# jamesonquinn/Mamba.jl

Hardware: AMD Instinct MI355X
Metric: chain-updates/sec (iters×chains) on rats model at 1/2/4/8 MI355X (higher is better)
Workload: dtype f64

## Files before the change

### mamba.jl_amd/csrc/device.h

```cpp
#pragma once
#if !defined(__HIPCC_RTC__)
#include <hip/hip_runtime.h>
#include <stdint.h>
#endif

#include "mamba_hip.h"
#include "mmb_math.h"
#include "ir_math.h"

#define MMB_MAXB MMB_MAX_BLOCKS

__device__ __forceinline__ bool mmb_inverse_ballot(uint64_t m) {
#if defined(__HIPCC_RTC__)
  return ((m >> (threadIdx.x & 63)) & 1ull) != 0ull;
#else
  return __builtin_amdgcn_inverse_ballot_w64(m);
#endif
}

template <bool B>
struct mmb_bc {
  static constexpr bool value = B;
  constexpr operator bool() const { return B; }
};
// ... 38 lines not shown
  double* t_accept;
  int32_t* t_m;
  int32_t* t_flags;
  double* t_Mv;
  double* t_Mvv;
  double* t_Ls;
  uint8_t* t_piv;
  double* t_xnext;
  int64_t* t_xtag;
  uint64_t* t_astat;
  double* t_nuts;
  double* t_nfr;
  double* t_hmc;
  int32_t ir_blk;
  int32_t fdgrad;
  const int32_t* sep;
  double sep_eps;
  int32_t gibbs_fam;
  double gibbs_a;
};

struct SweepArgs {
  int32_t K;
  uint32_t chain_offset;
  uint64_t seed;
  int64_t iter0;
  int32_t n_iters;
  int32_t nb;
  int64_t burnin, thin, model_burnin;
  int64_t kept_base;
  int64_t kept_origin;
  double* vals;
  int64_t xepoch;
  unsigned long long* nuts_stat;
  double* draws;
  const double* data0;
  double ig_c;
  double xbar;
  double xm[5];
  double lx[5], ly[5];
  const DBlock* blocks;
  const mmb_ir_node* ir_nodes;
  const int32_t* ir_code;
  const double* ir_const;
  const double* ir_pool;
  const mmb_ir_block* ir_blocks;
  const int32_t* ir_mon;
  int32_t ir_nmon, ir_pmon;
  int32_t ir_vs;
  int32_t ir_red0;
  int32_t ir_amm;
  int32_t ir_lds;
  const int32_t* cperm;
  int32_t amwg_exact;
  int32_t slice_exact;
  int32_t amwg_probe;
};

#define MMB_ORDER_BLOCKS 3
struct OrderArgs {
  const int32_t* flags[MMB_ORDER_BLOCKS];
  int32_t nblk;
  int32_t K;
  int32_t cpw;
  int32_t mode;
  int32_t* perm;
};

__device__ __forceinline__ const DBlock& mmb_block(const DBlock* p, int b) {
#if defined(__HIP_DEVICE_COMPILE__)
  return *(const DBlock*)&((const __attribute__((address_space(4))) DBlock*)p)[b];
#else
  return p[b];
#endif
}

MMB_HD int mmb_tri(int i) { return (i * (i + 1)) >> 1; }
MMB_HD int mmb_slot(int i, int k) { return i >= k ? mmb_tri(i) + k : mmb_tri(k) + i; }

__device__ __forceinline__ void grp_sync() {
  __builtin_amdgcn_fence(__ATOMIC_RELEASE, "wavefront");
  __builtin_amdgcn_wave_barrier();
  __builtin_amdgcn_fence(__ATOMIC_ACQUIRE, "wavefront");
}

template <int CTRL>
__device__ __forceinline__ int dpp_i(int x) {
  return __builtin_amdgcn_mov_dpp(x, CTRL, 0xF, 0xF, true);
}
template <int CTRL>
__device__ __forceinline__ double dpp_d(double x) {
  uint64_t u = mmb_d2u(x);
  int lo = dpp_i<CTRL>((int)(uint32_t)u), hi = dpp_i<CTRL>((int)(uint32_t)(u >> 32));
  return mmb_u2d((uint64_t)(uint32_t)lo | ((uint64_t)(uint32_t)hi << 32));
}
__device__ __forceinline__ int swap16_i(int x) {
  auto r = __builtin_amdgcn_permlane16_swap((unsigned)x, (unsigned)x, false, false);
  return (int)((threadIdx.x & 16) ? r[0] : r[1]);
}
__device__ __forceinline__ double swap16_d(double x) {
  uint64_t u = mmb_d2u(x);
  int lo = swap16_i((int)(uint32_t)u), hi = swap16_i((int)(uint32_t)(u >> 32));
  return mmb_u2d((uint64_t)(uint32_t)lo | ((uint64_t)(uint32_t)hi << 32));
}
template <int N, bool FIRST>
__device__ __forceinline__ void fmac_rowbc(double& acc, double x, double b) {
// ... 176 lines not shown
```

### mamba.jl_amd/csrc/engine.cpp

```cpp
#include <hip/hip_runtime.h>

#include <algorithm>
#include <cmath>
#include <cstdarg>
#include <cstdio>
#include <cstdlib>
#include <cstring>
#include <map>
#include <string>
#include <type_traits>
#include <vector>

#include "device.h"
#include "models.h"
#include "nuts.h"
#include "logistic.h"
#include "ir.h"
#include "ir_jit.h"

#include <rccl/rccl.h>

hipError_t mmb_launch_sweep(int model, unsigned kinds, const SweepArgs& A, hipStream_t st);
hipError_t mmb_launch_order_chains(const OrderArgs& a, hipStream_t st);
hipError_t mmb_launch_pchol_probe(int n, int d, const double* S, double* L, int32_t* pos, int32_t* info,
                                  hipStream_t st);
hipError_t mmb_lg_launch_ctl(const LgArgs& A, int start, int parity, int nbound, int fold, hipStream_t st);
hipError_t mmb_lg_launch_grad(const LgArgs& A, int parity, int nbound, int fold, hipStream_t st);
hipError_t mmb_launch_gr_range(int pmon, int64_t n, int K, const double* draws, double* out,
                               hipStream_t st);
hipError_t mmb_launch_chain_summary(int P, int64_t n, int K, int64_t kg0, int64_t bs, const double* draws,
                                    const double* shift, double* out, hipStream_t st);
hipError_t mmb_launch_order_hist(int P, int j, int64_t n, int K, const double* draws, int nt,
                                 const uint64_t* prefix, int pass, unsigned long long* counts, hipStream_t st);
hipError_t mmb_launch_gr_stats(int pmon, int64_t n, int K, const double* draws, const int32_t* link,
                               const double* shift, double* stats, hipStream_t st);

static thread_local std::string g_last_error;

struct BlockHost {
  mmb_block_spec spec;
  std::vector<double> tuning;
  int d = 0, T = 0, tune_len = 0;
  std::vector<double> sigl;
  bool sigl_diag = false;
  double *sigma = nullptr, *accept = nullptr, *Mv = nullptr, *Mvv = nullptr, *Ls = nullptr;
  double *nuts = nullptr, *nfr = nullptr, *width = nullptr, *sigl_d = nullptr;
  double* hmc = nullptr;
  int32_t *m = nullptr, *flags = nullptr;
  uint8_t* piv = nullptr;
  double* xnext = nullptr;
  int64_t* xtag = nullptr;
  uint64_t* astat = nullptr;
  int32_t* sep_d = nullptr;
  double sep_eps = 0.0;
};

struct mmb_engine {
  mmb_model_spec spec{};
  int device = 0;
  hipStream_t stream = nullptr;
  int model = 0;
  int P = 0, pmon = 0, VS = 0, DP = 0, TP = 0;
  std::vector<BlockHost> blocks;
  unsigned kinds = 0;
  std::vector<double> x, y, X;
  bool have_data = false;
  double* d_data = nullptr;
  int64_t K = 0, chain_offset = 0;
  uint64_t seed = 0;
  int64_t iter = 0;
  double* d_vals = nullptr;
  DBlock* d_blocks = nullptr;
  int lg_N = 0, lg_p = 0, lg_rps = 0;
  bool lg_fd = false;
  double *lg_X = nullptr, *lg_y = nullptr;
  double *lg_vec = nullptr, *lg_sc = nullptr, *lg_frames = nullptr, *lg_pos = nullptr;
  double *lg_gpart = nullptr, *lg_lpart = nullptr;
  int32_t *lg_iv = nullptr, *lg_count = nullptr, *lg_hcount = nullptr, *lg_s2c = nullptr;
  int64_t* lg_itc = nullptr;
  hipEvent_t lg_cev[2 * MMB_LG_SPLIT_MAX] = {};
  hipStream_t lg_streamx[MMB_LG_SPLIT_MAX - 1] = {};
  hipEvent_t lg_join[MMB_LG_SPLIT_MAX] = {};
  std::vector<hipEvent_t> evpoolx[MMB_LG_SPLIT_MAX - 1];
  int64_t lg_steps = 0;
  unsigned long long* lg_ngrad = nullptr;
  int32_t* d_cperm = nullptr;
  bool cperm_identity = true;
  bool order_fresh = false;
  int64_t order_iter = 0;
  unsigned long long* d_nstat = nullptr;
  unsigned long long slice_overflows = 0;
  int64_t xepoch = 0;
  double* d_draws = nullptr;
  size_t draws_cap = 0;
  int64_t n_kept = 0;
  std::vector<mmb_ir_node> ir_nodes;
  std::vector<int32_t> ir_code, ir_mon;
  std::vector<double> ir_const, ir_pool;
  std::vector<mmb_ir_block> ir_blocks;
  int ir_stack = 0;
  mmb_ir_node* d_ir_nodes = nullptr;
  int32_t *d_ir_code = nullptr, *d_ir_mon = nullptr;
  double *d_ir_const = nullptr, *d_ir_pool = nullptr;
  mmb_ir_block* d_ir_blocks = nullptr;
  hipModule_t jit_mod = nullptr;
  hipFunction_t jit_fn = nullptr;
  bool ir_noprop = false;
  int ir_stack_dbl = 0;
  std::string jit_info;
  hipEvent_t ev0 = nullptr, ev1 = nullptr;
  std::vector<hipEvent_t> evpool;
  double kernel_ms = 0.0;
  int64_t launches = 0, units = 0;
  std::string err;
};

static int fail(mmb_engine* e, int code, const char* fmt, ...) {
  char buf[512];
  va_list ap;
  va_start(ap, fmt);
  vsnprintf(buf, sizeof buf, fmt, ap);
  va_end(ap);
  g_last_error = buf;
  if (e) e->err = buf;
  return code;
}

#define HIPCHK(e, call)                                                                  \
  do {                                                                                   \
    hipError_t _st = (call);                                                             \
    if (_st != hipSuccess)                                                               \
      return fail((e), MMB_E_HIP, "%s failed: %s", #call, hipGetErrorString(_st));       \
  } while (0)

static int node_dim(const mmb_model_spec& s, const mmb_ir_model* ir, int node, bool* positive) {
  bool pos = false;
  int d = -1;
  if (s.model == MMB_MODEL_IR) {
// ... 598 lines not shown
}

int mmb_ir_jit_info(const mmb_engine* e, char* buf, int64_t n) {
  if (!e) return fail(nullptr, MMB_E_ARG, "null argument");
  if (buf && n > 0) snprintf(buf, (size_t)n, "%s", e->model == MMB_MODEL_IR ? e->jit_info.c_str() : "not a node-IR engine");
  return e->jit_fn ? 1 : 0;
}

static void free_dev(mmb_engine* e) {
  for (auto& h : e->blocks) {
    void* ptrs[] = {h.sigma, h.accept, h.Mv, h.Mvv, h.Ls, h.nuts, h.nfr, h.width, h.sigl_d, h.hmc, h.m, h.flags,
                    h.piv, h.xnext, h.xtag, h.astat};
    for (void* p : ptrs)
      if (p) (void)hipFree(p);
    h.sigma = h.accept = h.Mv = h.Mvv = h.Ls = h.nuts = h.nfr = h.width = h.sigl_d = h.hmc = nullptr;
    h.m = h.flags = nullptr;
    h.piv = nullptr;
    h.xnext = nullptr;
    h.xtag = nullptr;
    h.astat = nullptr;
  }
  if (e->d_vals) (void)hipFree(e->d_vals);
  if (e->d_blocks) (void)hipFree(e->d_blocks);
  {
    void* lp[] = {e->lg_vec, e->lg_sc, e->lg_frames, e->lg_pos, e->lg_gpart, e->lg_lpart, e->lg_iv,
                  e->lg_count, e->lg_itc, e->lg_s2c};
    for (void* q : lp)
      if (q) (void)hipFree(q);
    e->lg_vec = e->lg_sc = e->lg_frames = e->lg_pos = e->lg_gpart = e->lg_lpart = nullptr;
    e->lg_iv = e->lg_count = e->lg_s2c = nullptr;
    e->lg_itc = nullptr;
    if (e->lg_ngrad) (void)hipFree(e->lg_ngrad);
    e->lg_ngrad = nullptr;
    if (e->d_nstat) (void)hipFree(e->d_nstat);
    e->d_nstat = nullptr;
    if (e->d_cperm) (void)hipFree(e->d_cperm);
    e->d_cperm = nullptr;
    e->cperm_identity = true;
    e->order_fresh = false;
  }
  if (e->d_draws) (void)hipFree(e->d_draws);
  e->d_vals = nullptr;
  e->d_blocks = nullptr;
  e->d_draws = nullptr;
  e->draws_cap = 0;
}

#ifdef MMB_PHASE_PROF
void mmb_prof_dump();
void mmb_prof_dump_line();
#endif
#ifdef MMB_WAVE_TIMES
void mmb_wave_times_dump(int nwaves, int slots);
#endif

void mmb_destroy(mmb_engine* e) {
  if (!e) return;
  (void)hipSetDevice(e->device);
  if (e->stream) (void)hipStreamSynchronize(e->stream);
#ifdef MMB_WAVE_TIMES
  if (e->model == MMB_MODEL_RATS) mmb_wave_times_dump((int)((e->K + 1) / 2), 4096);
#endif
  if (e->jit_mod && std::getenv("MMB_IR_JIT_PROF") && std::atoi(std::getenv("MMB_IR_JIT_PROF")) == 1) {
    hipDeviceptr_t p = nullptr;
    size_t nb = 0;
    unsigned long long h[32] = {};
    if (hipModuleGetGlobal(&p, &nb, e->jit_mod, "mmb_prof") == hipSuccess && nb >= sizeof h &&
        hipMemcpyDtoH(h, p, sizeof h) == hipSuccess) {
      const char* names[] = {"-", "amm:load m/fl/Mv", "amm:proposal", "amm:logf x2+accept", "amm:moments+Sigma",
                             "amm:pchol", "amm:store", "gibbs", "iteration", "count", "pchol:steps",
                             "pchol:carry", "pchol:writeback", "amwg", "slice"};
      for (int i = 1; i < 15; ++i) fprintf(stderr, "MMB_PROF %-22s %llu\n", names[i], h[i]);
    }
  }
#ifdef MMB_PHASE_PROF
  mmb_prof_dump();
  mmb_prof_dump_line();
#endif
  free_dev(e);
  if (e->d_data) (void)hipFree(e->d_data);
  {
    void* ip[] = {e->d_ir_nodes, e->d_ir_code, e->d_ir_mon, e->d_ir_const, e->d_ir_pool, e->d_ir_blocks};
    for (void* q : ip)
      if (q) (void)hipFree(q);
    for (BlockHost& h : e->blocks)
      if (h.sep_d) (void)hipFree(h.sep_d);
  }
  if (e->lg_X) (void)hipFree(e->lg_X);
  if (e->lg_y) (void)hipFree(e->lg_y);
  if (e->lg_hcount) (void)hipHostFree(e->lg_hcount);
  for (hipEvent_t ev : e->lg_cev)
    if (ev) (void)hipEventDestroy(ev);
  for (hipEvent_t ev : e->lg_join)
    if (ev) (void)hipEventDestroy(ev);
  for (auto& pool : e->evpoolx)
    for (hipEvent_t ev : pool) (void)hipEventDestroy(ev);
  for (hipStream_t q : e->lg_streamx)
    if (q) (void)hipStreamDestroy(q);
  if (e->ev0) (void)hipEventDestroy(e->ev0);
  if (e->ev1) (void)hipEventDestroy(e->ev1);
  for (hipEvent_t ev : e->evpool) (void)hipEventDestroy(ev);
  if (e->stream) (void)hipStreamDestroy(e->stream);
  if (e->jit_mod) (void)hipModuleUnload(e->jit_mod);
  delete e;
}

int mmb_set_data(mmb_engine* e, const char* name, const double* x, int64_t n) {
  if (!e || !name || !x) return fail(e, MMB_E_ARG, "null argument");
  std::string nm(name);
  if (e->model == MMB_MODEL_LINE) {
    if (n != 5) return fail(e, MMB_E_ARG, "line: %s must have 5 elements", name);
    if (nm == "x") e->x.assign(x, x + 5);
    else if (nm == "y") e->y.assign(x, x + 5);
    else return fail(e, MMB_E_ARG, "line: unknown input %s", name);
  } else if (e->model == MMB_MODEL_LOGISTIC) {
    if (nm == "X") {
      if (n != (int64_t)e->lg_N * e->lg_p) return fail(e, MMB_E_ARG, "logistic: X must be nobs x ncoef");
      e->X.assign(x, x + n);
    } else if (nm == "y") {
      if (n != e->lg_N) return fail(e, MMB_E_ARG, "logistic: y must have nobs elements");
      for (int64_t i = 0; i < n; ++i)
        if (!(x[i] == 0.0 || x[i] == 1.0)) return fail(e, MMB_E_ARG, "logistic: y must be 0/1");
      e->y.assign(x, x + n);
    } else {
      return fail(e, MMB_E_ARG, "logistic: unknown input %s", name);
    }
    e->have_data = !e->X.empty() && !e->y.empty();
    if (e->have_data) {
      const size_t Np = (size_t)MMB_LG_NG * MMB_LG_NS * e->lg_rps;
      std::vector<double> hx(Np * MMB_LG_DV, 0.0), hy(Np, 0.0);
      for (int i = 0; i < e->lg_N; ++i) {
        for (int k = 0; k < e->lg_p; ++k) {
          hx[(size_t)i * MMB_LG_DV + k] = e->X[(size_t)i * e->lg_p + k];
        }
        hy[i] = e->y[i];
      }
      HIPCHK(e, hipSetDevice(e->device));
      if (!e->lg_X) HIPCHK(e, hipMalloc(&e->lg_X, hx.size() * sizeof(double)));
      if (!e->lg_y) HIPCHK(e, hipMalloc(&e->lg_y, hy.size() * sizeof(double)));
      HIPCHK(e, hipMemcpy(e->lg_X, hx.data(), hx.size() * sizeof(double), hipMemcpyHostToDevice));
      HIPCHK(e, hipMemcpy(e->lg_y, hy.data(), hy.size() * sizeof(double), hipMemcpyHostToDevice));
    }
    return 0;
  } else if (e->model == MMB_MODEL_RATS) {
    if (nm == "y") {
      if (n != 150) return fail(e, MMB_E_ARG, "rats: y must have 150 elements");
      e->y.assign(x, x + 150);
    } else if (nm == "x") {
      if (n != 5) return fail(e, MMB_E_ARG, "rats: x must have 5 elements");
      e->x.assign(x, x + 5);
// ... 205 lines not shown
      HIPCHK(e, hipMemcpy(h.hmc, t.data(), t.size() * sizeof(double), hipMemcpyHostToDevice));
      if (!h.sigl.empty()) {
        HIPCHK(e, dalloc(&h.sigl_d, (size_t)h.d * h.d));
        HIPCHK(e, hipMemcpy(h.sigl_d, h.sigl.data(), h.sigl.size() * sizeof(double), hipMemcpyHostToDevice));
      }
    } else if (h.spec.sampler == MMB_SAMPLER_SLICE && h.tuning.size() > 1) {
      HIPCHK(e, dalloc(&h.width, h.tuning.size()));
      HIPCHK(e, hipMemcpy(h.width, h.tuning.data(), h.tuning.size() * sizeof(double), hipMemcpyHostToDevice));
    }
  }
  if (e->model == MMB_MODEL_LOGISTIC) {
    HIPCHK(e, dalloc(&e->lg_vec, (size_t)K * MMB_LG_NVEC * MMB_LG_DV));
    HIPCHK(e, hipMemset(e->lg_vec, 0, (size_t)K * MMB_LG_NVEC * MMB_LG_DV * sizeof(double)));
    HIPCHK(e, dalloc(&e->lg_sc, (size_t)K * MMB_LG_NSC));
    HIPCHK(e, dalloc(&e->lg_iv, (size_t)K * MMB_LG_NIV));
    HIPCHK(e, hipMemset(e->lg_iv, 0, (size_t)K * MMB_LG_NIV * sizeof(int32_t)));
    HIPCHK(e, dalloc(&e->lg_itc, (size_t)K));
    HIPCHK(e, dalloc(&e->lg_frames, (size_t)K * NutsFrames<MMB_LG_DV>::DBL));
    HIPCHK(e, dalloc(&e->lg_pos, (size_t)K * MMB_LG_DV));
    HIPCHK(e, dalloc(&e->lg_gpart, (size_t)MMB_LG_NG * MMB_LG_NS * K * MMB_LG_DV));
    HIPCHK(e, dalloc(&e->lg_lpart, (size_t)MMB_LG_NG * MMB_LG_NS * K * (e->lg_fd ? e->lg_p + 1 : 1)));
    HIPCHK(e, dalloc(&e->lg_count, 2 * MMB_LG_SPLIT_MAX));
    HIPCHK(e, dalloc(&e->lg_s2c, (size_t)2 * K));
    HIPCHK(e, dalloc(&e->lg_ngrad, 1));
    if (!e->lg_hcount) HIPCHK(e, hipHostMalloc(&e->lg_hcount, 2 * MMB_LG_SPLIT_MAX * sizeof(int32_t), 0));
    for (hipEvent_t& ev : e->lg_cev)
      if (!ev) HIPCHK(e, hipEventCreateWithFlags(&ev, hipEventDisableTiming));
    for (hipEvent_t& ev : e->lg_join)
      if (!ev) HIPCHK(e, hipEventCreateWithFlags(&ev, hipEventDisableTiming));
    for (hipStream_t& q : e->lg_streamx)
      if (!q) HIPCHK(e, hipStreamCreateWithFlags(&q, hipStreamNonBlocking));
  }
  int rc = upload_blocks(e);
  if (rc) return rc;
  return mmb_set_values(e, init);
}

static int64_t kept_upto(int64_t t, int64_t burnin, int64_t thin) {
  return t > burnin ? (t - burnin) / thin : 0;
}

static void fill_args(const mmb_engine* e, SweepArgs& A) {
  std::memset(&A, 0, sizeof A);
  A.K = (int32_t)e->K;
  A.chain_offset = (uint32_t)e->chain_offset;
  A.seed = e->seed;
  A.nb = (int32_t)e->blocks.size();
  A.vals = e->d_vals;
  A.xepoch = e->xepoch;
  A.nuts_stat = e->d_nstat;
  A.ig_c = 0.001 * std::log(0.001) - std::lgamma(0.001);
  A.blocks = e->d_blocks;
  A.cperm = e->cperm_identity ? nullptr : e->d_cperm;
  {
    const char* ae = std::getenv("MMB_AMWG_EXACT");
    const int v = ae ? std::atoi(ae) : 0;
    A.amwg_exact = (v == 1 || v == 2) ? v : 0;
    const char* se = std::getenv("MMB_SLICE_EXACT");
    A.slice_exact = (se && std::atoi(se) == 1) ? 1 : 0;
    const char* ap = std::getenv("MMB_AMWG_PROBE");
    A.amwg_probe = (ap && std::atoi(ap) == 1) ? 1 : 0;
  }
  if (e->model == MMB_MODEL_IR) {
    A.ir_nodes = e->d_ir_nodes; A.ir_code = e->d_ir_code; A.ir_const = e->d_ir_const;
    A.ir_pool = e->d_ir_pool; A.ir_blocks = e->d_ir_blocks; A.ir_mon = e->d_ir_mon;
    A.ir_nmon = (int32_t)e->ir_mon.size();
    A.ir_pmon = e->pmon;
    A.ir_vs = e->VS;
    A.ir_red0 = e->P;
    A.ir_amm = (e->kinds & (1u << MMB_SAMPLER_AMM)) ? (int32_t)(e->TP + 4 * Mdl<MMB_MODEL_IR>::DP + 2) : 0;
    A.ir_lds = A.ir_amm + (e->ir_noprop ? 1 : 2) * e->VS +
               (e->jit_fn ? e->ir_stack_dbl : (e->ir_stack + 1) * Mdl<MMB_MODEL_IR>::G);
  } else if (e->model == MMB_MODEL_RATS) {
    double s = 0.0;
    for (int i = 0; i < 5; ++i) s += e->x[i];
    A.xbar = s / 5.0;
    for (int i = 0; i < 5; ++i) A.xm[i] = e->x[i] - A.xbar;
    A.data0 = e->d_data;
  } else {
    for (int i = 0; i < 5; ++i) { A.lx[i] = e->x[i]; A.ly[i] = e->y[i]; }
  }
}

static int iters_per_launch(const mmb_engine* e) {
  const char* s = std::getenv("MMB_ITERS_PER_LAUNCH");
  if (s && std::atoi(s) > 0) return std::atoi(s);
  return e->model == MMB_MODEL_RATS ? 20 : e->model == MMB_MODEL_IR ? 16 : e->model == MMB_MODEL_LINE ? 256 : 64;
}

template <class T>
static int d2h(mmb_engine* e, std::vector<T>& h, const T* d, size_t n) {
  h.resize(n);
  HIPCHK(e, hipMemcpy(h.data(), d, n * sizeof(T), hipMemcpyDeviceToHost));
  return 0;
}
template <class T>
static int h2d(mmb_engine* e, T* d, const std::vector<T>& h) {
  HIPCHK(e, hipMemcpy(d, h.data(), h.size() * sizeof(T), hipMemcpyHostToDevice));
  return 0;
}

static int order_chains(mmb_engine* e) {
  e->cperm_identity = true;
  if (!(e->model == MMB_MODEL_RATS || e->model == MMB_MODEL_IR) || e->K < 4) return 0;
  const char* env = std::getenv("MMB_ORDER_CHAINS");
  if (env && std::string(env) == "0") return 0;
  OrderArgs oa;
  std::memset(&oa, 0, sizeof oa);
  for (const BlockHost& h : e->blocks)
    if (h.spec.sampler == MMB_SAMPLER_AMM && h.flags && oa.nblk < MMB_ORDER_BLOCKS) oa.flags[oa.nblk++] = h.flags;
  if (oa.nblk == 0) return 0;
  if (!e->d_cperm) HIPCHK(e, dalloc(&e->d_cperm, (size_t)e->K));
  oa.K = (int32_t)e->K;
  oa.perm = e->d_cperm;
  oa.cpw = e->model == MMB_MODEL_RATS ? 8 : 4;
  {
    const char* om = std::getenv("MMB_ORDER_MODE");
    oa.mode = om ? std::atoi(om) : 1;
    if (oa.mode < 0 || oa.mode > 2) oa.mode = 1;
  }
  hipError_t st = mmb_launch_order_chains(oa, e->stream);
  if (st != hipSuccess) return fail(e, MMB_E_HIP, "order_chains launch: %s", hipGetErrorString(st));
  e->cperm_identity = false;
  return 0;
}

static int64_t order_every() {
  const char* s = std::getenv("MMB_ORDER_EVERY");
  return (s && std::atoi(s) > 0) ? std::atoi(s) : 64;
}

static int launch_width(int64_t iters, int W, int64_t li) {
  const int64_t nl = (iters + W - 1) / W;
  const int64_t q = iters / nl, r = iters % nl;
  return (int)(q + (li < r ? 1 : 0));
}


#ifndef MMB_LG_FOLD_MIN
#define MMB_LG_FOLD_MIN 1024
// ... 155 lines not shown
    e->launches = 0;
    for (int i = 0; i < nh; ++i) e->launches += H[i].s;
    e->units = a->iters * e->K;
  }
  e->iter += a->iters;
  e->n_kept = want ? nk : 0;
  if (a->draws && nk > 0) {
    std::vector<double> hd((size_t)nk * e->pmon * e->K);
    HIPCHK(e, hipMemcpyAsync(hd.data(), e->d_draws, hd.size() * sizeof(double), hipMemcpyDeviceToHost,
                             e->stream));
    HIPCHK(e, hipStreamSynchronize(e->stream));
    for (int64_t i = 0; i < nk; ++i)
      for (int j = 0; j < e->pmon; ++j)
        for (int64_t k = 0; k < e->K; ++k)
          a->draws[i + nk * (j + (int64_t)e->pmon * k)] = hd[(i * e->pmon + j) * e->K + k];
  }
  HIPCHK(e, hipStreamSynchronize(e->stream));
  return 0;
}

int mmb_run(mmb_engine* e, const mmb_run_args* a) {
  if (!e || !a) return fail(e, MMB_E_ARG, "null argument");
  if (!e->d_vals) return fail(e, MMB_E_STATE, "mmb_init_chains not called");
  if (a->iters < 0 || a->thin < 1 || a->burnin < 0)
    return fail(e, MMB_E_ARG, "iters >= 0, thin >= 1, burnin >= 0 required");
  if (e->iter + a->iters > 0xffffffffLL) return fail(e, MMB_E_ARG, "iteration counter overflow");
  HIPCHK(e, hipSetDevice(e->device));
  const int64_t it0 = e->iter;
  const int64_t kept0 = kept_upto(it0, a->burnin, a->thin);
  const int64_t nk = kept_upto(it0 + a->iters, a->burnin, a->thin) - kept0;
  const bool want = (a->draws != nullptr) || a->keep_device;
  if (want && nk > 0) {
    size_t need = (size_t)nk * e->pmon * e->K;
    if (need > e->draws_cap) {
      if (e->d_draws) HIPCHK(e, hipFree(e->d_draws));
      e->d_draws = nullptr;
      HIPCHK(e, dalloc(&e->d_draws, need));
      e->draws_cap = need;
    }
  }
  if (e->model == MMB_MODEL_LOGISTIC) return run_logistic(e, a, (want && nk > 0) ? e->d_draws : nullptr, kept0, nk, want);
  if (a->iters > 0 && !e->order_fresh) {
    int orc = order_chains(e);
    if (orc) return orc;
    e->order_iter = it0;
  }
  SweepArgs A;
  fill_args(e, A);
  A.burnin = a->burnin;
  A.thin = a->thin;
  A.model_burnin = a->model_burnin;
  A.kept_origin = kept0;
  A.draws = (want && nk > 0) ? e->d_draws : nullptr;
  const int W = iters_per_launch(e);
  e->kernel_ms = 0.0;
  e->launches = 0;
  e->units = 0;
  const int64_t nl = (a->iters + W - 1) / W;
  if (a->time_kernels) {
    while ((int64_t)e->evpool.size() < 2 * nl) {
      hipEvent_t ev;
      HIPCHK(e, hipEventCreate(&ev));
      e->evpool.push_back(ev);
    }
  }
  for (int64_t done = 0, li = 0, w = 0; done < a->iters; done += w, ++li) {
    w = launch_width(a->iters, W, li);
    A.iter0 = it0 + done;
    A.n_iters = w;
    if (a->time_kernels) HIPCHK(e, hipEventRecord(e->evpool[2 * li], e->stream));
    hipError_t st;
    if (e->jit_fn) {
      const int per_block = 128 / Mdl<MMB_MODEL_IR>::G;
      const unsigned grid = (unsigned)((A.K + per_block - 1) / per_block);
      const size_t lds = (size_t)per_block * Mdl<MMB_MODEL_IR>::lds_stride(A) * sizeof(double);
      void* args[] = {(void*)&A};
      st = hipModuleLaunchKernel(e->jit_fn, grid, 1, 1, 128, 1, 1, (unsigned)lds, e->stream, args, nullptr);
    } else {
      st = mmb_launch_sweep(e->model, e->kinds, A, e->stream);
    }
    if (st != hipSuccess) return fail(e, MMB_E_HIP, "sweep launch: %s", hipGetErrorString(st));
    if (a->time_kernels) HIPCHK(e, hipEventRecord(e->evpool[2 * li + 1], e->stream));
    e->launches += 1;
    e->units += (int64_t)w * e->K;
  }
  if (a->iters > 0 && (!e->order_fresh || it0 + a->iters - e->order_iter >= order_every())) {
    int orc = order_chains(e);
    if (orc) return orc;
    e->order_fresh = true;
    e->order_iter = it0 + a->iters;
  }
  if (a->time_kernels) {
    HIPCHK(e, hipEventSynchronize(e->evpool[2 * nl - 1]));
    for (int64_t li = 0; li < nl; ++li) {
      float ms = 0.f;
      HIPCHK(e, hipEventElapsedTime(&ms, e->evpool[2 * li], e->evpool[2 * li + 1]));
      e->kernel_ms += ms;
    }
  }
  e->iter = it0 + a->iters;
  e->n_kept = want ? nk : 0;
  if ((e->kinds & (1u << MMB_SAMPLER_SLICE)) && a->iters > 0) {
    unsigned long long ov = 0;
    HIPCHK(e, hipMemcpyAsync(&ov, e->d_nstat + 3, sizeof ov, hipMemcpyDeviceToHost, e->stream));
    HIPCHK(e, hipStreamSynchronize(e->stream));
    if (ov != e->slice_overflows) {
      const unsigned long long n = ov - e->slice_overflows;
      e->slice_overflows = ov;
      return fail(e, MMB_E_STATE, "Slice: %llu update(s) in iterations %lld..%lld still rejected after %d shrink "
                  "steps (the reference would loop forever; check the widths and the target's support)",
                  n, (long long)it0 + 1, (long long)e->iter, MMB_SLICE_MAX_SHRINK);
    }
  }
  if (a->draws && nk > 0) {
    std::vector<double> h((size_t)nk * e->pmon * e->K);
    HIPCHK(e, hipMemcpyAsync(h.data(), e->d_draws, h.size() * sizeof(double), hipMemcpyDeviceToHost,
                             e->stream));
    HIPCHK(e, hipStreamSynchronize(e->stream));
    for (int64_t i = 0; i < nk; ++i)
      for (int j = 0; j < e->pmon; ++j)
        for (int64_t k = 0; k < e->K; ++k)
          a->draws[i + nk * (j + (int64_t)e->pmon * k)] = h[(i * e->pmon + j) * e->K + k];
  }
  return 0;
}

int mmb_reserve_draws(mmb_engine* e, int64_t nkept) {
  if (!e || nkept < 0) return fail(e, MMB_E_ARG, "null engine or nkept < 0");
  if (!e->d_vals) return fail(e, MMB_E_STATE, "mmb_init_chains not called");
  const size_t need = (size_t)nkept * e->pmon * e->K;
  if (need > e->draws_cap) {
    HIPCHK(e, hipSetDevice(e->device));
    HIPCHK(e, hipStreamSynchronize(e->stream));
    if (e->d_draws) HIPCHK(e, hipFree(e->d_draws));
    e->d_draws = nullptr;
    e->draws_cap = 0;
    e->n_kept = 0;
    HIPCHK(e, dalloc(&e->d_draws, need));
    e->draws_cap = need;
  }
  return 0;
}

int mmb_get_draws(mmb_engine* e, double* draws) {
  if (!e || !draws) return fail(e, MMB_E_ARG, "null argument");
  const int64_t nk = e->n_kept;
  if (nk == 0) return 0;
  std::vector<double> h((size_t)nk * e->pmon * e->K);
  HIPCHK(e, hipSetDevice(e->device));
  HIPCHK(e, hipStreamSynchronize(e->stream));
// ... 623 lines not shown
```

### mamba.jl_amd/csrc/sweep.h

```cpp
#pragma once
#include "samplers.h"
#include "ir.h"

#ifdef MMB_PHASE_PROF
extern __device__ unsigned long long mmb_prof[32];
#endif
#ifdef MMB_WAVE_TIMES
#define MMB_WT_MAX 65536
extern __device__ unsigned long long mmb_wt[2 * MMB_WT_MAX];
#endif

#ifndef MMB_SWEEP_WAVES
#define MMB_SWEEP_WAVES 4
#endif
#ifndef MMB_IR_WAVES
#define MMB_IR_WAVES 2
#endif
template <int MODEL>
constexpr int sweep_waves() {
  return MODEL == MMB_MODEL_RATS ? MMB_SWEEP_WAVES : MODEL == MMB_MODEL_IR ? MMB_IR_WAVES : 1;
}

template <int MODEL, unsigned KINDS>
__device__ __forceinline__ void sweep_body(const SweepArgs& A) {
  using M = Mdl<MODEL>;
  using S = Smp<M>;
  constexpr int G = M::G;
  extern __shared__ __attribute__((aligned(16))) double smem[];
  if constexpr ((KINDS >> MMB_SAMPLER_AMM) & 1u) {
    S::ik_fill();
    __syncthreads();
  }
#ifdef MMB_IR_POOL_LDS
  if constexpr (MODEL == MMB_MODEL_IR) {
    double* ps = mmb_ir_pool_s();
    for (int t = (int)threadIdx.x; t < MMB_IR_POOL_LDS; t += (int)blockDim.x) ps[t] = A.ir_pool[t];
    __syncthreads();
  }
#endif
  const int slot = (int)((blockIdx.x * blockDim.x + threadIdx.x) / G);
#ifdef MMB_WAVE_TIMES
  const uint64_t _wt0 = __builtin_amdgcn_s_memrealtime();
  const int _wid = (int)((blockIdx.x * blockDim.x + threadIdx.x) >> 6);
#endif
  if (slot >= A.K) return;
  const int c = A.cperm != nullptr ? A.cperm[slot] : slot;
  Grp<G> g;
  double* lds = smem + (size_t)(threadIdx.x / G) * M::lds_stride(A);
  typename M::St s;
  typename M::Lc l;
  M::load(A, c, g.lane, s, l, lds);
  const uint32_t chain = A.chain_offset + (uint32_t)c;
#ifdef MMB_PHASE_PROF
  if ((threadIdx.x & 63) == 0)
    for (int i = 0; i < 16; ++i) mmb_prof_lds()[i] = 0;
#endif
  for (int step = 0; step < A.n_iters; ++step) {
    const int64_t it = A.iter0 + 1 + step;
#ifdef MMB_PHASE_PROF
    const uint64_t _it0 = __builtin_amdgcn_s_memtime();
#endif
    double pre = 0.0;
    if constexpr (G == 32 && (KINDS & ((1u << MMB_SAMPLER_GIBBS) | (1u << MMB_SAMPLER_AMM))) != 0u)
      pre = S::predraw(A, chain, it, g);
    for (int b = 0; b < A.nb; ++b) {
      const DBlock& B = mmb_block(A.blocks, b);
      const mmb_rng rn = mmb_rng_make(A.seed, chain, (uint32_t)it, (uint32_t)b, MMB_SUB_NORMAL);
      const mmb_rng ru = mmb_rng_make(A.seed, chain, (uint32_t)it, (uint32_t)b, MMB_SUB_UNIFORM);
      const bool adapt = B.adapt == MMB_ADAPT_ALL ? true
                         : B.adapt == MMB_ADAPT_BURNIN ? (it <= A.model_burnin) : false;
      switch (B.kind) {
        case MMB_SAMPLER_AMWG:
          if constexpr ((KINDS >> MMB_SAMPLER_AMWG) & 1u) {
            MMB_PROF_START
            S::amwg(A, B, c, rn, ru, adapt, s, l, g);
            MMB_PROF_MARK(13, g.lane)
          }
          break;
        case MMB_SAMPLER_AMM:
          if constexpr ((KINDS >> MMB_SAMPLER_AMM) & 1u) S::amm(A, B, c, chain, it, b, rn, ru, adapt, s, l, g, lds,
                                                                        G == 32 ? S::lane_value(pre, b) : 0.0);
          break;
        case MMB_SAMPLER_SLICE:
          if constexpr ((KINDS >> MMB_SAMPLER_SLICE) & 1u) {
            MMB_PROF_START
            if (B.form == MMB_SLICE_UNIVARIATE) S::slice_uni(A, B, ru, s, l, g, lds);
            else S::slice_multi(A, B, ru, s, l, g, lds);
            MMB_PROF_MARK(14, g.lane)
          }
          break;
        case MMB_SAMPLER_NUTS:
          if constexpr ((KINDS >> MMB_SAMPLER_NUTS) & 1u) S::nuts(A, B, c, it, b, s, g);
          break;
        case MMB_SAMPLER_HMC:
          if constexpr ((KINDS >> MMB_SAMPLER_HMC) & 1u) S::template hmc<false>(A, B, c, rn, ru, s, g);
          break;
        case MMB_SAMPLER_MALA:
          if constexpr ((KINDS >> MMB_SAMPLER_MALA) & 1u) S::template hmc<true>(A, B, c, rn, ru, s, g);
          break;
        case MMB_SAMPLER_GIBBS: if constexpr ((KINDS >> MMB_SAMPLER_GIBBS) & 1u) {
          const mmb_rng gn = mmb_rng_make(A.seed, chain, (uint32_t)it, (uint32_t)b, MMB_SUB_GAMMA_N);
          const mmb_rng gu = mmb_rng_make(A.seed, chain, (uint32_t)it, (uint32_t)b, MMB_SUB_GAMMA_U);
          MMB_PROF_START
          M::gibbs(A, B, s, l, g, &rn, &gn, &gu, G == 32 ? S::lane_value(pre, b) : 0.0);
          MMB_PROF_MARK(7, g.lane)
        }
          break;
        default:
          break;
      }
    }
#ifdef MMB_PHASE_PROF
    if ((threadIdx.x & 63) == 0) {
      mmb_prof_lds()[8] += __builtin_amdgcn_s_memtime() - _it0;
      mmb_prof_lds()[9] += 1;
    }
#endif
    if (A.draws && it > A.burnin && (it - A.burnin) % A.thin == 0) {
      const int64_t row = (it - A.burnin) / A.thin - 1 - A.kept_origin;
      M::write_draws(A, s, g, row, c);
    }
  }
  M::store(A, c, g.lane, s);
#ifdef MMB_WAVE_TIMES
  if ((threadIdx.x & 63) == 0 && _wid < MMB_WT_MAX) {
    mmb_wt[2 * _wid] = _wt0;
    mmb_wt[2 * _wid + 1] = __builtin_amdgcn_s_memrealtime();
  }
#endif
#ifdef MMB_PHASE_PROF
  if ((threadIdx.x & 63) == 0)
    for (int i = 0; i < 16; ++i) atomicAdd(&mmb_prof[i], mmb_prof_lds()[i]);
#endif
}

#ifndef MMB_RATS_BLOCK
#define MMB_RATS_BLOCK 256
#endif
template <int MODEL, unsigned KINDS>
__global__ __launch_bounds__(MODEL == MMB_MODEL_RATS && MMB_RATS_BLOCK > 256 ? MMB_RATS_BLOCK : 256,
                             sweep_waves<MODEL>()) void sweep_kernel(const SweepArgs A) {
  sweep_body<MODEL, KINDS>(A);
}

constexpr unsigned K_ALL = (1u << MMB_SAMPLER_AMWG) | (1u << MMB_SAMPLER_AMM) |
                         (1u << MMB_SAMPLER_SLICE) | (1u << MMB_SAMPLER_GIBBS);
constexpr unsigned K_GRAD = (1u << MMB_SAMPLER_NUTS) | (1u << MMB_SAMPLER_HMC) | (1u << MMB_SAMPLER_MALA);
constexpr unsigned K_ALL_GRAD = K_ALL | K_GRAD;
constexpr unsigned K_GIBBS_AMM = (1u << MMB_SAMPLER_AMM) | (1u << MMB_SAMPLER_GIBBS);
constexpr unsigned K_SLICE_AMWG = (1u << MMB_SAMPLER_AMWG) | (1u << MMB_SAMPLER_SLICE);
constexpr unsigned K_IR = (1u << MMB_SAMPLER_AMWG) | (1u << MMB_SAMPLER_AMM) | (1u << MMB_SAMPLER_SLICE) |
                         (1u << MMB_SAMPLER_GIBBS) | K_GRAD;
```

### mamba.jl_amd/csrc/sweep.hip

```cpp
#include "sweep.h"
#include <cstdlib>

#ifdef MMB_PHASE_PROF
#include <cstdio>
__device__ unsigned long long mmb_prof[32];
void mmb_prof_dump() {
  unsigned long long h[32];
  if (hipMemcpyFromSymbol(h, HIP_SYMBOL(mmb_prof), sizeof h) != hipSuccess) return;
  const char* names[] = {"-", "amm:load m/fl/Mv", "amm:proposal", "amm:logf x2+accept", "amm:moments+Sigma",
                         "amm:pchol", "amm:store", "gibbs", "iteration", "count", "pchol:steps",
                         "pchol:carry", "pchol:writeback", "amwg", "slice", "-"};
  for (int i = 1; i < 15; ++i) fprintf(stderr, "MMB_PROF %-22s %llu\n", names[i], h[i]);
}
#endif

#ifdef MMB_WAVE_TIMES
#include <algorithm>
#include <cstdio>
#include <vector>
__device__ unsigned long long mmb_wt[2 * MMB_WT_MAX];
void mmb_wave_times_dump(int nwaves, int slots) {
  std::vector<unsigned long long> h(2 * MMB_WT_MAX);
  if (hipMemcpyFromSymbol(h.data(), HIP_SYMBOL(mmb_wt), h.size() * sizeof(unsigned long long)) != hipSuccess) return;
  nwaves = std::min(nwaves, MMB_WT_MAX);
  unsigned long long t0 = ~0ull, t1 = 0;
  double busy = 0.0;
  int n = 0;
  for (int w = 0; w < nwaves; ++w) {
    if (h[2 * w] == 0 || h[2 * w + 1] < h[2 * w]) continue;
    t0 = std::min(t0, h[2 * w]);
    t1 = std::max(t1, h[2 * w + 1]);
    busy += (double)(h[2 * w + 1] - h[2 * w]);
    ++n;
  }
  if (!n) return;
  const double span = (double)(t1 - t0);
  int dec[10] = {0}, sdec[10] = {0};
  for (int w = 0; w < nwaves; ++w) {
    if (h[2 * w] == 0) continue;
    dec[std::min(9, (int)(10.0 * (double)(h[2 * w + 1] - t0) / span))]++;
    sdec[std::min(9, (int)(10.0 * (double)(h[2 * w] - t0) / span))]++;
  }
  fprintf(stderr, "MMB_WT waves %d span_us %.1f mean_wave_us %.1f fill(slots=%d) %.4f\nMMB_WT end_deciles", n,
          span / 100.0, busy / n / 100.0, slots, busy / (span * slots));
  for (int i = 0; i < 10; ++i) fprintf(stderr, " %d", dec[i]);
  fprintf(stderr, "\nMMB_WT start_deciles");
  for (int i = 0; i < 10; ++i) fprintf(stderr, " %d", sdec[i]);
  fprintf(stderr, "\n");
}
#endif

template <int MODEL, unsigned KINDS>
static hipError_t launch(const SweepArgs& A, hipStream_t st, int threads) {
  using M = Mdl<MODEL>;
  const int per_block = threads / M::G;
  const int blocks = (A.K + per_block - 1) / per_block;
  const size_t lds = (size_t)per_block * M::lds_stride(A) * sizeof(double);
  hipLaunchKernelGGL((sweep_kernel<MODEL, KINDS>), dim3(blocks), dim3(threads), lds, st, A);
  return hipGetLastError();
}

constexpr int ORD_T = 1024;
constexpr int ORD_KC = 16384;
__global__ __launch_bounds__(ORD_T) void order_chains_kernel(const OrderArgs a) {
  __shared__ int32_t cnt[(1 << MMB_ORDER_BLOCKS) * ORD_T];
  __shared__ int32_t wsum[ORD_T / 64];
  __shared__ uint8_t ccls[ORD_KC];
  const int t = (int)threadIdx.x;
  const int NC = 1 << a.nblk;
  const int C = (a.K + ORD_T - 1) / ORD_T;
  const int k0 = min(a.K, t * C), k1 = min(a.K, k0 + C);
  auto gcls = [&](int k) {
    int c = 0;
    for (int b = 0; b < a.nblk; ++b) c = (c << 1) | ((a.flags[b][k] >> 2) & 1);
    return c;
  };
  const bool cached = a.K <= ORD_KC;
  if (cached) {
    for (int k = t; k < a.K; k += ORD_T) ccls[k] = (uint8_t)gcls(k);
    __syncthreads();
  }
  auto cls = [&](int k) { return cached ? (int)ccls[k] : gcls(k); };
  for (int c = 0; c < NC; ++c) cnt[c * ORD_T + t] = 0;
  for (int k = k0; k < k1; ++k) cnt[cls(k) * ORD_T + t] += 1;
  __syncthreads();
  int* own = cnt + t * NC;
  int s = 0;
  for (int i = 0; i < NC; ++i) s += own[i];
  const int lane = t & 63, w = t >> 6;
  int inc = s;
  for (int d = 1; d < 64; d <<= 1) {
    const int v = __shfl_up(inc, d, 64);
    if (lane >= d) inc += v;
  }
  if (lane == 63) wsum[w] = inc;
  __syncthreads();
  int base = 0;
  for (int i = 0; i < w; ++i) base += wsum[i];
  int run = base + inc - s;
  __syncthreads();
  for (int i = 0; i < NC; ++i) {
    const int v = own[i];
    own[i] = run;
    run += v;
  }
  __syncthreads();
  const int W = a.cpw / 2, NF = a.K / a.cpw;
  for (int k = k0; k < k1; ++k) {
    int* p = &cnt[cls(k) * ORD_T + t];
    int pos = *p;
    *p += 1;
    if (a.mode == 1) pos = a.K - 1 - pos;
    if (a.mode == 2 && W > 0 && (pos >> 1) < NF * W) {
      const int q = pos >> 1;
      pos = (q % NF) * a.cpw + 2 * (q / NF) + (pos & 1);
    }
    a.perm[pos] = k;
  }
}

hipError_t mmb_launch_order_chains(const OrderArgs& a, hipStream_t st) {
  if (a.nblk < 1 || a.nblk > MMB_ORDER_BLOCKS || a.K < 1) return hipErrorInvalidValue;
  hipLaunchKernelGGL(order_chains_kernel, dim3(1), dim3(ORD_T), 0, st, a);
  return hipGetLastError();
}

hipError_t mmb_launch_line_amm(const SweepArgs& A, hipStream_t st);

hipError_t mmb_launch_sweep(int model, unsigned kinds, const SweepArgs& A, hipStream_t st) {
  if (model == MMB_MODEL_RATS) {
    constexpr int TB = MMB_RATS_BLOCK;
    if ((kinds & ~K_GIBBS_AMM) == 0) return launch<MMB_MODEL_RATS, K_GIBBS_AMM>(A, st, TB);
    if ((kinds & ~K_SLICE_AMWG) == 0) return launch<MMB_MODEL_RATS, K_SLICE_AMWG>(A, st, TB);
    return launch<MMB_MODEL_RATS, K_ALL>(A, st, TB);
  }
  if (model == MMB_MODEL_IR) return launch<MMB_MODEL_IR, K_IR>(A, st, 128);
  if (model == MMB_MODEL_LINE) {
    if (kinds == (1u << MMB_SAMPLER_AMM) && A.nb == 1 && !std::getenv("MMB_LINE_GENERIC"))
      return mmb_launch_line_amm(A, st);
    if (kinds & K_GRAD) return launch<MMB_MODEL_LINE, K_ALL_GRAD>(A, st, 64);
    return launch<MMB_MODEL_LINE, K_ALL>(A, st, 64);
  }
  return hipErrorInvalidValue;
}
```

Baseline: 129.7 million.

## Split sweep launches into interleaved workgroup partitions across concurrent streams

The sweep grid is split into up to two interleaved workgroup subsets (wg_offset/wg_stride), each launched on its own non-blocking stream, with events forking from and joining back to the main stream. The aim is to let one partition's tail overlap the next launch of the other partition, reducing the idle slots caused by stragglers at kernel boundaries. Iterations per launch are capped at half the requested iterations when split. The split is used only when each part still fills the device's resident workgroup capacity. Kernel timing now merges overlapping intervals, and the wave-timing instrumentation accumulates busy time per slot.

After: 144.6 million (median of 6 runs). +11.5%, better.

```diff
diff --git a/mamba.jl_amd/csrc/device.h b/mamba.jl_amd/csrc/device.h
--- a/mamba.jl_amd/csrc/device.h
+++ b/mamba.jl_amd/csrc/device.h
@@ -114,6 +114,8 @@
   int32_t ir_amm;
   int32_t ir_lds;
   const int32_t* cperm;
+  int32_t wg_offset;
+  int32_t wg_stride;
   int32_t amwg_exact;
   int32_t slice_exact;
   int32_t amwg_probe;
diff --git a/mamba.jl_amd/csrc/engine.cpp b/mamba.jl_amd/csrc/engine.cpp
--- a/mamba.jl_amd/csrc/engine.cpp
+++ b/mamba.jl_amd/csrc/engine.cpp
@@ -35,7 +35,11 @@
 hipError_t mmb_launch_gr_stats(int pmon, int64_t n, int K, const double* draws, const int32_t* link,
                                const double* shift, double* stats, hipStream_t st);
 
+hipError_t mmb_sweep_shape(int model, unsigned kinds, const SweepArgs& A, int* nwg, int* wg_per_cu);
+
 static thread_local std::string g_last_error;
+
+constexpr int MMB_SWEEP_PARTS_MAX = 4;
 
 struct BlockHost {
   mmb_block_spec spec;
@@ -84,6 +88,10 @@
   std::vector<hipEvent_t> evpoolx[MMB_LG_SPLIT_MAX - 1];
   int64_t lg_steps = 0;
   unsigned long long* lg_ngrad = nullptr;
+  hipStream_t sw_streamx[MMB_SWEEP_PARTS_MAX - 1] = {};
+  hipEvent_t sw_join[MMB_SWEEP_PARTS_MAX] = {};
+  std::vector<hipEvent_t> sw_evpoolx[MMB_SWEEP_PARTS_MAX - 1];
+  int sw_resident = 0;
   int32_t* d_cperm = nullptr;
   bool cperm_identity = true;
   bool order_fresh = false;
@@ -788,6 +796,7 @@
 #endif
 #ifdef MMB_WAVE_TIMES
 void mmb_wave_times_dump(int nwaves, int slots);
+void mmb_wave_times_reset(hipStream_t st);
 #endif
 
 void mmb_destroy(mmb_engine* e) {
@@ -795,7 +804,8 @@
   (void)hipSetDevice(e->device);
   if (e->stream) (void)hipStreamSynchronize(e->stream);
 #ifdef MMB_WAVE_TIMES
-  if (e->model == MMB_MODEL_RATS) mmb_wave_times_dump((int)((e->K + 1) / 2), 4096);
+  if (e->model == MMB_MODEL_RATS)
+    mmb_wave_times_dump((int)((e->K + 1) / 2), e->sw_resident > 0 ? 4 * e->sw_resident : 4096);
 #endif
   if (e->jit_mod && std::getenv("MMB_IR_JIT_PROF") && std::atoi(std::getenv("MMB_IR_JIT_PROF")) == 1) {
     hipDeviceptr_t p = nullptr;
@@ -832,6 +842,12 @@
   for (auto& pool : e->evpoolx)
     for (hipEvent_t ev : pool) (void)hipEventDestroy(ev);
   for (hipStream_t q : e->lg_streamx)
+    if (q) (void)hipStreamDestroy(q);
+  for (hipEvent_t ev : e->sw_join)
+    if (ev) (void)hipEventDestroy(ev);
+  for (auto& pool : e->sw_evpoolx)
+    for (hipEvent_t ev : pool) (void)hipEventDestroy(ev);
+  for (hipStream_t q : e->sw_streamx)
     if (q) (void)hipStreamDestroy(q);
   if (e->ev0) (void)hipEventDestroy(e->ev0);
   if (e->ev1) (void)hipEventDestroy(e->ev1);
@@ -1143,6 +1159,8 @@
   A.ig_c = 0.001 * std::log(0.001) - std::lgamma(0.001);
   A.blocks = e->d_blocks;
   A.cperm = e->cperm_identity ? nullptr : e->d_cperm;
+  A.wg_offset = 0;
+  A.wg_stride = 1;
   {
     const char* ae = std::getenv("MMB_AMWG_EXACT");
     const int v = ae ? std::atoi(ae) : 0;
@@ -1173,10 +1191,49 @@
   }
 }
 
-static int iters_per_launch(const mmb_engine* e) {
+constexpr int MMB_SWEEP_PARTS_DEFAULT = 2;
+static int sweep_parts(mmb_engine* e, const SweepArgs& A, int* parts) {
+  *parts = 1;
+  if (!(e->model == MMB_MODEL_RATS || e->model == MMB_MODEL_IR)) return 0;
+  int nwg = 0, per_cu = 0;
+  if (e->jit_fn) {
+    const int per_block = 128 / Mdl<MMB_MODEL_IR>::G;
+    nwg = (A.K + per_block - 1) / per_block;
+    if (!e->sw_resident) {
+      const size_t lds = (size_t)per_block * Mdl<MMB_MODEL_IR>::lds_stride(A) * sizeof(double);
+      HIPCHK(e, hipModuleOccupancyMaxActiveBlocksPerMultiprocessor(&per_cu, e->jit_fn, 128, lds));
+    }
+  } else {
+    hipError_t st = mmb_sweep_shape(e->model, e->kinds, A, &nwg, e->sw_resident ? nullptr : &per_cu);
+    if (st != hipSuccess) return fail(e, MMB_E_HIP, "sweep shape: %s", hipGetErrorString(st));
+  }
+  if (!e->sw_resident) {
+    int cus = 0;
+    HIPCHK(e, hipDeviceGetAttribute(&cus, hipDeviceAttributeMultiprocessorCount, e->device));
+    e->sw_resident = std::max(1, per_cu * cus);
+  }
+  int p = 1;
+  const char* s = std::getenv("MMB_SWEEP_PARTS");
+  if (s && std::atoi(s) >= 1) {
+    p = std::min(std::atoi(s), MMB_SWEEP_PARTS_MAX);
+  } else {
+    p = MMB_SWEEP_PARTS_DEFAULT;
+    while (p > 1 && nwg / p < e->sw_resident) --p;
+  }
+  *parts = std::max(1, std::min(p, nwg));
+  return 0;
+}
+
+static int iters_per_launch_one(const mmb_engine* e) {
+  return e->model == MMB_MODEL_RATS ? 20 : e->model == MMB_MODEL_IR ? 16 : e->model == MMB_MODEL_LINE ? 256 : 64;
+}
+
+static int iters_per_launch(const mmb_engine* e, int parts, int64_t iters) {
   const char* s = std::getenv("MMB_ITERS_PER_LAUNCH");
   if (s && std::atoi(s) > 0) return std::atoi(s);
-  return e->model == MMB_MODEL_RATS ? 20 : e->model == MMB_MODEL_IR ? 16 : e->model == MMB_MODEL_LINE ? 256 : 64;
+  const int W = iters_per_launch_one(e);
+  if (parts > 1 && iters > 1) return (int)std::min<int64_t>(W, (iters + 1) / 2);
+  return W;
 }
 
 template <class T>
@@ -1438,50 +1495,110 @@
   A.model_burnin = a->model_burnin;
   A.kept_origin = kept0;
   A.draws = (want && nk > 0) ? e->d_draws : nullptr;
-  const int W = iters_per_launch(e);
+  int np = 1;
+  {
+    int rc = sweep_parts(e, A, &np);
+    if (rc) return rc;
+  }
+  const int W = iters_per_launch(e, np, a->iters);
   e->kernel_ms = 0.0;
   e->launches = 0;
   e->units = 0;
-  const int64_t nl = (a->iters + W - 1) / W;
-  if (a->time_kernels) {
-    while ((int64_t)e->evpool.size() < 2 * nl) {
-      hipEvent_t ev;
-      HIPCHK(e, hipEventCreate(&ev));
-      e->evpool.push_back(ev);
-    }
+  const int64_t nl = a->iters > 0 ? (a->iters + W - 1) / W : 0;
+  hipStream_t pst[MMB_SWEEP_PARTS_MAX];
+  std::vector<hipEvent_t>* pev[MMB_SWEEP_PARTS_MAX];
+  for (int p = 0; p < np; ++p) {
+    if (p > 0 && !e->sw_streamx[p - 1])
+      HIPCHK(e, hipStreamCreateWithFlags(&e->sw_streamx[p - 1], hipStreamNonBlocking));
+    pst[p] = p == 0 ? e->stream : e->sw_streamx[p - 1];
+    pev[p] = p == 0 ? &e->evpool : &e->sw_evpoolx[p - 1];
+    if (a->time_kernels) {
+      while ((int64_t)pev[p]->size() < 2 * nl) {
+        hipEvent_t ev;
+        HIPCHK(e, hipEventCreate(&ev));
+        pev[p]->push_back(ev);
+      }
+    }
+  }
+  if (np > 1)
+    for (int p = 0; p < np; ++p)
+      if (!e->sw_join[p]) HIPCHK(e, hipEventCreateWithFlags(&e->sw_join[p], hipEventDisableTiming));
+  struct PartDrain {
+    hipStream_t* st;
+    int n;
+    bool armed = true;
+    ~PartDrain() {
+      if (armed)
+        for (int p = 1; p < n; ++p) (void)hipStreamSynchronize(st[p]);
+    }
+  } drain{pst, np};
+#ifdef MMB_WAVE_TIMES
+  if (nl > 0) mmb_wave_times_reset(e->stream);
+#endif
+  if (np > 1 && nl > 0) {
+    HIPCHK(e, hipEventRecord(e->sw_join[0], e->stream));
+    for (int p = 1; p < np; ++p) HIPCHK(e, hipStreamWaitEvent(pst[p], e->sw_join[0], 0));
   }
   for (int64_t done = 0, li = 0, w = 0; done < a->iters; done += w, ++li) {
     w = launch_width(a->iters, W, li);
     A.iter0 = it0 + done;
     A.n_iters = w;
-    if (a->time_kernels) HIPCHK(e, hipEventRecord(e->evpool[2 * li], e->stream));
-    hipError_t st;
-    if (e->jit_fn) {
-      const int per_block = 128 / Mdl<MMB_MODEL_IR>::G;
-      const unsigned grid = (unsigned)((A.K + per_block - 1) / per_block);
-      const size_t lds = (size_t)per_block * Mdl<MMB_MODEL_IR>::lds_stride(A) * sizeof(double);
-      void* args[] = {(void*)&A};
-      st = hipModuleLaunchKernel(e->jit_fn, grid, 1, 1, 128, 1, 1, (unsigned)lds, e->stream, args, nullptr);
-    } else {
-      st = mmb_launch_sweep(e->model, e->kinds, A, e->stream);
-    }
-    if (st != hipSuccess) return fail(e, MMB_E_HIP, "sweep launch: %s", hipGetErrorString(st));
-    if (a->time_kernels) HIPCHK(e, hipEventRecord(e->evpool[2 * li + 1], e->stream));
-    e->launches += 1;
+    for (int p = 0; p < np; ++p) {
+      A.wg_offset = p;
+      A.wg_stride = np;
+      if (a->time_kernels) HIPCHK(e, hipEventRecord((*pev[p])[2 * li], pst[p]));
+      hipError_t st;
+      if (e->jit_fn) {
+        const int per_block = 128 / Mdl<MMB_MODEL_IR>::G;
+        const int nwg = (A.K + per_block - 1) / per_block;
+        const unsigned grid = (unsigned)((nwg - p + np - 1) / np);
+        const size_t lds = (size_t)per_block * Mdl<MMB_MODEL_IR>::lds_stride(A) * sizeof(double);
+        void* args[] = {(void*)&A};
+        st = hipModuleLaunchKernel(e->jit_fn, grid, 1, 1, 128, 1, 1, (unsigned)lds, pst[p], args, nullptr);
+      } else {
+        st = mmb_launch_sweep(e->model, e->kinds, A, pst[p]);
+      }
+      if (st != hipSuccess) return fail(e, MMB_E_HIP, "sweep launch: %s", hipGetErrorString(st));
+      if (a->time_kernels) HIPCHK(e, hipEventRecord((*pev[p])[2 * li + 1], pst[p]));
+      e->launches += 1;
+    }
     e->units += (int64_t)w * e->K;
   }
+  if (np > 1 && nl > 0) {
+    for (int p = 1; p < np; ++p) {
+      HIPCHK(e, hipEventRecord(e->sw_join[p], pst[p]));
+      HIPCHK(e, hipStreamWaitEvent(e->stream, e->sw_join[p], 0));
+    }
+  }
+  drain.armed = false;
   if (a->iters > 0 && (!e->order_fresh || it0 + a->iters - e->order_iter >= order_every())) {
     int orc = order_chains(e);
     if (orc) return orc;
     e->order_fresh = true;
     e->order_iter = it0 + a->iters;
   }
-  if (a->time_kernels) {
-    HIPCHK(e, hipEventSynchronize(e->evpool[2 * nl - 1]));
-    for (int64_t li = 0; li < nl; ++li) {
-      float ms = 0.f;
-      HIPCHK(e, hipEventElapsedTime(&ms, e->evpool[2 * li], e->evpool[2 * li + 1]));
-      e->kernel_ms += ms;
+  if (a->time_kernels && nl > 0) {
+    std::vector<std::pair<float, float>> iv;
+    for (int p = 0; p < np; ++p) {
+      HIPCHK(e, hipEventSynchronize((*pev[p])[2 * nl - 1]));
+      for (int64_t li = 0; li < nl; ++li) {
+        float t0 = 0.f, dt = 0.f;
+        HIPCHK(e, hipEventElapsedTime(&dt, (*pev[p])[2 * li], (*pev[p])[2 * li + 1]));
+        if (np == 1) {
+          e->kernel_ms += dt;
+          continue;
+        }
+        if (p > 0 || li > 0) HIPCHK(e, hipEventElapsedTime(&t0, (*pev[0])[0], (*pev[p])[2 * li]));
+        iv.emplace_back(t0, t0 + dt);
+      }
+    }
+    std::sort(iv.begin(), iv.end());
+    for (size_t i = 0; i < iv.size();) {
+      float hi = iv[i].second;
+      size_t j = i + 1;
+      for (; j < iv.size() && iv[j].first <= hi; ++j) hi = std::max(hi, iv[j].second);
+      e->kernel_ms += hi - iv[i].first;
+      i = j;
     }
   }
   e->iter = it0 + a->iters;
diff --git a/mamba.jl_amd/csrc/sweep.h b/mamba.jl_amd/csrc/sweep.h
--- a/mamba.jl_amd/csrc/sweep.h
+++ b/mamba.jl_amd/csrc/sweep.h
@@ -7,7 +7,7 @@
 #endif
 #ifdef MMB_WAVE_TIMES
 #define MMB_WT_MAX 65536
-extern __device__ unsigned long long mmb_wt[2 * MMB_WT_MAX];
+extern __device__ unsigned long long mmb_wt[3 * MMB_WT_MAX];
 #endif
 
 #ifndef MMB_SWEEP_WAVES
@@ -38,10 +38,11 @@
     __syncthreads();
   }
 #endif
-  const int slot = (int)((blockIdx.x * blockDim.x + threadIdx.x) / G);
+  const unsigned wg = blockIdx.x * (unsigned)A.wg_stride + (unsigned)A.wg_offset;
+  const int slot = (int)((wg * blockDim.x + threadIdx.x) / G);
 #ifdef MMB_WAVE_TIMES
   const uint64_t _wt0 = __builtin_amdgcn_s_memrealtime();
-  const int _wid = (int)((blockIdx.x * blockDim.x + threadIdx.x) >> 6);
+  const int _wid = (int)((wg * blockDim.x + threadIdx.x) >> 6);
 #endif
   if (slot >= A.K) return;
   const int c = A.cperm != nullptr ? A.cperm[slot] : slot;
@@ -124,8 +125,10 @@
   M::store(A, c, g.lane, s);
 #ifdef MMB_WAVE_TIMES
   if ((threadIdx.x & 63) == 0 && _wid < MMB_WT_MAX) {
-    mmb_wt[2 * _wid] = _wt0;
-    mmb_wt[2 * _wid + 1] = __builtin_amdgcn_s_memrealtime();
+    const uint64_t _wt1 = __builtin_amdgcn_s_memrealtime();
+    if (mmb_wt[3 * _wid] == 0) mmb_wt[3 * _wid] = _wt0;
+    mmb_wt[3 * _wid + 1] = _wt1;
+    mmb_wt[3 * _wid + 2] += _wt1 - _wt0;
   }
 #endif
 #ifdef MMB_PHASE_PROF
diff --git a/mamba.jl_amd/csrc/sweep.hip b/mamba.jl_amd/csrc/sweep.hip
--- a/mamba.jl_amd/csrc/sweep.hip
+++ b/mamba.jl_amd/csrc/sweep.hip
@@ -18,35 +18,30 @@
 #include <algorithm>
 #include <cstdio>
 #include <vector>
-__device__ unsigned long long mmb_wt[2 * MMB_WT_MAX];
+__device__ unsigned long long mmb_wt[3 * MMB_WT_MAX];
+void mmb_wave_times_reset(hipStream_t st) {
+  void* p = nullptr;
+  if (hipGetSymbolAddress(&p, HIP_SYMBOL(mmb_wt)) == hipSuccess)
+    (void)hipMemsetAsync(p, 0, sizeof(unsigned long long) * 3 * MMB_WT_MAX, st);
+}
 void mmb_wave_times_dump(int nwaves, int slots) {
-  std::vector<unsigned long long> h(2 * MMB_WT_MAX);
+  std::vector<unsigned long long> h(3 * MMB_WT_MAX);
   if (hipMemcpyFromSymbol(h.data(), HIP_SYMBOL(mmb_wt), h.size() * sizeof(unsigned long long)) != hipSuccess) return;
   nwaves = std::min(nwaves, MMB_WT_MAX);
   unsigned long long t0 = ~0ull, t1 = 0;
   double busy = 0.0;
   int n = 0;
   for (int w = 0; w < nwaves; ++w) {
-    if (h[2 * w] == 0 || h[2 * w + 1] < h[2 * w]) continue;
-    t0 = std::min(t0, h[2 * w]);
-    t1 = std::max(t1, h[2 * w + 1]);
-    busy += (double)(h[2 * w + 1] - h[2 * w]);
+    if (h[3 * w] == 0 || h[3 * w + 1] < h[3 * w]) continue;
+    t0 = std::min(t0, h[3 * w]);
+    t1 = std::max(t1, h[3 * w + 1]);
+    busy += (double)h[3 * w + 2];
     ++n;
   }
   if (!n) return;
   const double span = (double)(t1 - t0);
-  int dec[10] = {0}, sdec[10] = {0};
-  for (int w = 0; w < nwaves; ++w) {
-    if (h[2 * w] == 0) continue;
-    dec[std::min(9, (int)(10.0 * (double)(h[2 * w + 1] - t0) / span))]++;
-    sdec[std::min(9, (int)(10.0 * (double)(h[2 * w] - t0) / span))]++;
-  }
-  fprintf(stderr, "MMB_WT waves %d span_us %.1f mean_wave_us %.1f fill(slots=%d) %.4f\nMMB_WT end_deciles", n,
+  fprintf(stderr, "MMB_WT window: wave slots %d span_us %.1f busy_per_slot_us %.1f fill(slots=%d) %.4f\n", n,
           span / 100.0, busy / n / 100.0, slots, busy / (span * slots));
-  for (int i = 0; i < 10; ++i) fprintf(stderr, " %d", dec[i]);
-  fprintf(stderr, "\nMMB_WT start_deciles");
-  for (int i = 0; i < 10; ++i) fprintf(stderr, " %d", sdec[i]);
-  fprintf(stderr, "\n");
 }
 #endif
 
@@ -54,10 +49,23 @@
 static hipError_t launch(const SweepArgs& A, hipStream_t st, int threads) {
   using M = Mdl<MODEL>;
   const int per_block = threads / M::G;
-  const int blocks = (A.K + per_block - 1) / per_block;
+  const int nwg = (A.K + per_block - 1) / per_block;
+  if (A.wg_stride < 1 || A.wg_offset < 0 || A.wg_offset >= A.wg_stride) return hipErrorInvalidValue;
+  const int blocks = (nwg - A.wg_offset + A.wg_stride - 1) / A.wg_stride;
+  if (blocks <= 0) return hipSuccess;
   const size_t lds = (size_t)per_block * M::lds_stride(A) * sizeof(double);
   hipLaunchKernelGGL((sweep_kernel<MODEL, KINDS>), dim3(blocks), dim3(threads), lds, st, A);
   return hipGetLastError();
+}
+
+template <int MODEL, unsigned KINDS>
+static hipError_t shape(const SweepArgs& A, int threads, int* nwg, int* wg_per_cu) {
+  using M = Mdl<MODEL>;
+  const int per_block = threads / M::G;
+  *nwg = (A.K + per_block - 1) / per_block;
+  if (!wg_per_cu) return hipSuccess;
+  const size_t lds = (size_t)per_block * M::lds_stride(A) * sizeof(double);
+  return hipOccupancyMaxActiveBlocksPerMultiprocessor(wg_per_cu, sweep_kernel<MODEL, KINDS>, threads, lds);
 }
 
 constexpr int ORD_T = 1024;
@@ -143,3 +151,14 @@
   }
   return hipErrorInvalidValue;
 }
+
+hipError_t mmb_sweep_shape(int model, unsigned kinds, const SweepArgs& A, int* nwg, int* wg_per_cu) {
+  if (model == MMB_MODEL_RATS) {
+    constexpr int TB = MMB_RATS_BLOCK;
+    if ((kinds & ~K_GIBBS_AMM) == 0) return shape<MMB_MODEL_RATS, K_GIBBS_AMM>(A, TB, nwg, wg_per_cu);
+    if ((kinds & ~K_SLICE_AMWG) == 0) return shape<MMB_MODEL_RATS, K_SLICE_AMWG>(A, TB, nwg, wg_per_cu);
+    return shape<MMB_MODEL_RATS, K_ALL>(A, TB, nwg, wg_per_cu);
+  }
+  if (model == MMB_MODEL_IR) return shape<MMB_MODEL_IR, K_IR>(A, 128, nwg, wg_per_cu);
+  return hipErrorInvalidValue;
+}
```
